# JuliaGaussianProcesses/ApproximateGPs.jl

Hardware: NVIDIA B200
Metric: SVGP ELBO+grad points/sec (FP64) (higher is better)
Workload: dtype f64

## Files before the change

approximategps.jl_b200/csrc/agp.cu:

```cuda
#include <dlfcn.h>
#include <nccl.h>
#include <stdarg.h>
#include <stdio.h>
#include <string.h>

#include <algorithm>
#include <string>
#include <vector>

#include "../../include/agp.h"
#include "dense.cuh"
#include "f32sweep.cuh"
#include "gemm.cuh"
#include "kfun.cuh"
#include "laplace.cuh"
#include "sweep.cuh"

using namespace agp;

static thread_local std::string g_err;
static thread_local int32_t g_err_info = 0;
static int32_t fail(int32_t code, const char* fmt, ...) {
  char buf[1024];
  va_list ap;
// ... 525 lines not shown

template <int MODE>
static int32_t launch_trsm(agp_ctx* c, const TrsmArgs& a, int tiles_n) {
  if ((MODE == TR_KUF_FWD || MODE == TR_KUF_FWD_SCALED) && a.kp.D > 8) return launch_trsm_s<MODE, 3>(c, a, tiles_n);
  return launch_trsm_s<MODE, 4>(c, a, tiles_n);
}

template <int LA, int LB, int S = StageCfg<LA, LB>::stages, class Epi>
static int32_t run_gemm(agp_ctx* c, int tiles_m, int tiles_n, const double* A, int64_t lda, const double* B, int64_t ldb, int K,
                        int kmode, int tmode, const Epi& epi) {
  using Cfg = StageCfg<LA, LB>;
  constexpr int smem_bytes = S * Cfg::bytes;
  GemmArgs g{A, lda, B, ldb, K, kmode, tmode};
  OK((ensure_smem<gemm_kernel<LA, LB, Epi, S>>(c, smem_bytes)));
  dim3 grid(tiles_m, tiles_n);
  if ((kmode == KR_LOWER || kmode == KR_UPPER) && tmode == TS_ALL && tiles_m > 1) {
    static const int env_g = getenv("AGP_SWIZZLE") ? atoi(getenv("AGP_SWIZZLE")) : 0;
    g.swizzle = env_g > 0 ? env_g : std::max(1, c->sms);
    g.tiles_m = tiles_m;
    g.tiles_n = tiles_n;
    grid = dim3(tiles_m * tiles_n, 1);
  }
  gemm_kernel<LA, LB, Epi, S><<<grid, NTHREADS, smem_bytes, c->stream>>>(g, epi);
  LAUNCHED(c);
  KCHECK();
  return AGP_OK;
}

static EpiStore epi_store(double* C, int64_t ldc, bool rowmajor, double alpha = 1.0, double beta = 0.0, int mask = MASK_NONE,
                          double diag_add = 0.0, const double* u = nullptr, const double* v = nullptr, double r1 = 0.0) {
  EpiStore e;
  e.C = C;
  e.ldc = ldc;
  e.rowmajor = rowmajor ? 1 : 0;
  e.alpha = alpha;
  e.beta = beta;
  e.mask = mask;
  e.diag_add = diag_add;
  e.r1u = u;
  e.r1v = v;
  e.r1 = r1;
  return e;
}

static int32_t fill(agp_ctx* c, double* p, int64_t n, double v) {
  if (n <= 0) return AGP_OK;
// ... 976 lines not shown
    } else if (emu_s2 && ncols >= 2048) {
      ProfScope ps(c, PC_GEMM_BTA);
      const int64_t pbytes = (int64_t)Mp * ldc;
      OK(c->q6As.ensure(((int64_t)i8e::S * pbytes + 7) / 8));
      OK(c->sPm.ensure(ldc));
      signed char* qApm = reinterpret_cast<signed char*>(c->q6As.p);
      i8e::transpose_slice_kernel<i8e::S><<<(ncols + 31) / 32, 256, 0, c->stream>>>(c->A.p, ldc, Mp, ncols, qApm, Mp, pbytes, c->sPm.p);
      LAUNCHED(c);
      KCHECK();
      CUtensorMap ma, mb;
      if (!i8e::make_map3(&ma, qApm, Mp, ncols, Mp, pbytes, i8e::EM, i8e::S) ||
          !i8e::make_map3(&mb, reinterpret_cast<signed char*>(c->qBt7.p), Mp, Mp, Mp, MM, i8e::EN, i8e::S))
        return fail(AGP_ERR_CUDA, "cuTensorMapEncodeTiled failed");
      i8e::EpiE2 e2{c->C.p, ldc, c->sPm.p, c->sBt7.p, c->scc_part.p, ldc};
      i8e::Args g8{Mp, i8e::KM_FROM_N, 0, 0};
      OK((ensure_smem<i8e::i8emu_gemm_kernel<i8e::EpiE2>>(c, i8e::SMEM_BYTES)));
      i8e::i8emu_gemm_kernel<i8e::EpiE2><<<dim3(Mp / i8e::EN, ncols / i8e::EM, 1), i8e::E_THREADS, i8e::SMEM_BYTES, c->stream>>>(ma, mb, g8, e2);
      LAUNCHED(c);
      KCHECK();
    } else {
    EpiS2 e2{c->C.p, ldc, c->scc_part.p, ldc};
    {
      ProfScope ps(c, PC_GEMM_BTA);
      OK((run_gemm<A_KM, B_KN>(c, nb, tiles_n, c->Bt_rm.p, Mp, c->A.p, ldc, Mp, KR_UPPER, TS_ALL, e2)));
    }
    }
    PerPointArgs pp{};
    pp.saa = c->saa.p;
    pp.sam = c->sam.p;
    pp.scc_part = c->scc_part.p;
    pp.ldp = ldc;
    pp.nb = st.f32 ? 2 * nb : ((emu_s2 && ncols >= 2048) ? 4 * nb : nb);
    pp.pts = pts;
    pp.y = y ? y + lo : nullptr;
    pp.npts = npts;
    pp.ncols = ncols;
    pp.scale = st.scale;
    pp.mean_const = st.mean_const;
    pp.kp = st.kp;
    pp.lp = st.lp;
    pp.dmu = c->dmu.p;
    pp.dv = c->dv.p;
    pp.mu_out = mu_out ? mu_out + lo : nullptr;
    pp.var_out = var_out ? var_out + lo : nullptr;
    pp.sc_part = c->sc_part.p;
    pp.flag = c->d_flags + 1;
    pp.predict_only = predict ? 1 : 0;
// ... 61 lines not shown
        t5a.kp = st.kp;
        ProfScope ps(c, PC_TRSM_BWD);
        OK(launch_trsm<TR_RHS_BWD>(c, t5a, tiles_n));
      }
      {
        ProfScope ps(c, PC_SYRK);
        const int kchunk = (int)round_up((ncols + c->nsplit - 1) / c->nsplit, t5::TM);
        const int nz = (ncols + kchunk - 1) / kchunk;
        t5::EpiF6 e6{c->Gpart.p, Mp};
        t5::Args g{ncols, t5::KM_SPLIT, kchunk, 1, t5::MnDesc()};
        OK((launch_t5<true, true>(c, dim3(Mp / t5::TM, Mp / t5::TN, nz), fAs, plane, Mp, ncols, fA, plane, Mp, ncols, g, e6)));
      }
      {
        ProfScope ps(c, PC_F32_AUX);
        const int slab = 512, nslab = (ncols + slab - 1) / slab;
        t5::gvec_kernel<<<dim3((Mp / 4 + 255) / 256, nslab), 256, 0, c->stream>>>(fA, fA + plane, Mp, Mp, c->dmu.p, ncols, slab, c->gpart.p, Mp);
        LAUNCHED(c);
        KCHECK();
      }
    } else {
    EpiS4 e4{c->A.p, c->Ab.p, c->As.p, ldc, c->dmu.p, c->dv.p, c->mt.p, c->gpart.p, Mp};
    {
      ProfScope ps(c, PC_GEMM_BC);
      OK((run_gemm<A_KM, B_KN>(c, nb, tiles_n, c->Bt_cm.p, Mp, c->C.p, ldc, Mp, KR_LOWER, TS_ALL, e4)));
    }
    TrsmArgs t5a{};
    t5a.T = c->Ut.p;
    t5a.ldt = Mp;
    t5a.nb = nb;
    t5a.X = c->Ab.p;
    t5a.ldx = ldc;
    t5a.kp = st.kp;
    {
      ProfScope ps(c, PC_TRSM_BWD);
      OK(launch_trsm<TR_RHS_BWD>(c, t5a, tiles_n));
    }
    if (st.f64_emu && Mp >= 768 && ncols >= 2048) {
      ProfScope ps(c, PC_SYRK);
      const int64_t ldk = round_up(ncols, 128), pbytes = (int64_t)Mp * ldk;
      OK(c->q6A.ensure(((int64_t)i8e::S * pbytes + 7) / 8));
      OK(c->q6As.ensure(((int64_t)i8e::S * pbytes + 7) / 8));
      OK(c->s6.ensure(4 * (int64_t)Mp));
      double* sA = c->s6.p;
      double* sAs = c->s6.p + Mp;
      unsigned long long* mx = reinterpret_cast<unsigned long long*>(c->s6.p + 2 * Mp);
      CU(cudaMemsetAsync(mx, 0, sizeof(unsigned long long) * 2 * Mp, c->stream));
      const int seg = 8192;
// ... 8 lines not shown
      c->launches += 4;
      KCHECK();
      CUtensorMap ma, mb;
      if (!i8e::make_map3(&ma, qAs, ldk, Mp, ldk, pbytes, i8e::EM, i8e::S) || !i8e::make_map3(&mb, qA, ldk, Mp, ldk, pbytes, i8e::EN, i8e::S))
        return fail(AGP_ERR_CUDA, "cuTensorMapEncodeTiled failed");
      const int kchunk = 16384, nz = (int)((ldk + kchunk - 1) / kchunk);
      if (nz > c->nsplit) return fail(AGP_ERR_ALLOC, "S6 (INT8): %d slabs of G needed, %d allocated", nz, c->nsplit);
      i8e::EpiE6 e6{c->Gpart.p, Mp, sAs, sA};
      i8e::Args g8{(int)ldk, i8e::KM_SPLIT, kchunk, 1};
      OK((ensure_smem<i8e::i8emu_gemm_kernel<i8e::EpiE6>>(c, i8e::SMEM_BYTES)));
      i8e::i8emu_gemm_kernel<i8e::EpiE6><<<dim3(Mp / i8e::EN, Mp / i8e::EM, nz), i8e::E_THREADS, i8e::SMEM_BYTES, c->stream>>>(ma, mb, g8, e6);
      LAUNCHED(c);
      KCHECK();
    } else {
      ProfScope ps(c, PC_SYRK);
      SyrkArgs s{};
      s.As = c->As.p;
      s.A = c->A.p;
      s.ld = ldc;
      s.ncols = ncols;
      s.kchunk = (int)round_up((ncols + c->nsplit - 1) / c->nsplit, BK);
      s.G = c->Gpart.p;
      s.Mp = Mp;
      using Cfg = StageCfg<A_MK, B_NK>;
      OK((ensure_smem<syrk_kernel>(c, Cfg::smem_bytes)));
      dim3 grid(nb * (nb + 1), c->nsplit);
      syrk_kernel<<<grid, NTHREADS, Cfg::smem_bytes, c->stream>>>(s);
      LAUNCHED(c);
      KCHECK();
    }
    }
    {
      ProfScope ps(c, PC_KGRAD);
      if (kgrad_fast(st)) {
        OK(run_kgrad(c, c->Ab.p, ldc, pts, npts, (npts + 2047) / 2048, c->Kf.p, st.kp.kind != AGP_KERNEL_SE ? c->DKb.p : nullptr));
      } else {
        OK(run_kgrad(c, c->Ab.p, ldc, pts, npts, (npts + 2047) / 2048));
      }
    }
  }
  if (predict || !grad) return AGP_OK;
  sum_slices_kernel<<<(Mp + 255) / 256, 256, 0, c->stream>>>(c->gpart.p, (int)(ldc / BN), Mp, Mp, c->red.p + rl.g);
  LAUNCHED(c);
  KCHECK();
  sum_slices_kernel<<<1024, 256, 0, c->stream>>>(c->Gpart.p, c->nsplit, MM, MM, c->red.p + rl.G);
  LAUNCHED(c);
  KCHECK();
  OK(finish_kgrad(c, c->nslab, 1.0, c->red.p + rl.dZ, c->red.p + rl.theta));
  return AGP_OK;
}
// ... 339 lines not shown
  xbuf.release();
  if (s != AGP_OK) return s;
  if (e != cudaSuccess) return fail(AGP_ERR_CUDA, "mean_and_var: %s", cudaGetErrorString(e));
  return check_step_flags(c, false);
}

static int32_t project_points(agp_ctx* c, const double* X_dev, int n, int ncols, double* Abuf, double* Cbuf, int64_t ldc) {
  SvgpState& st = c->st;
  TrsmArgs t1{};
  t1.T = c->Lt.p;
  t1.ldt = st.Mp;
  t1.nb = st.nb;
  t1.X = Abuf;
  t1.ldx = ldc;
  t1.pts = X_dev;
  t1.npts = n;
  t1.zsp = c->zsp.p;
  t1.mt = c->mt.p;
  t1.saa = c->saa.p;
  t1.sam = c->sam.p;
  t1.kp = st.kp;
  OK(launch_s1(c, t1, ncols / BN));
  EpiS2 e2{Cbuf, ldc, c->scc_part.p, ldc};
  OK((run_gemm<A_KM, B_KN>(c, st.nb, ncols / BN, c->Bt_rm.p, st.Mp, Abuf, ldc, st.Mp, KR_UPPER, TS_ALL, e2)));
  return AGP_OK;
}

constexpr int64_t AGP_MAX_COV_POINTS = 16384;

extern "C" int32_t agp_svgp_mean_and_cov(agp_ctx* c, const agp_svgp_params* p, const double* X1, int64_t n1, const double* X2, int64_t n2,
                                         double* mu1_out, double* cov_out) {
  if (!c || !p || !X1 || n1 < 1 || !cov_out) return fail(AGP_ERR_INVALID, "agp_svgp_mean_and_cov: bad arguments");
  const bool cross = X2 != nullptr;
  if (!cross) n2 = n1;
  if (n2 < 1) return fail(AGP_ERR_INVALID, "agp_svgp_mean_and_cov: bad arguments");
  if (n1 > AGP_MAX_COV_POINTS || n2 > AGP_MAX_COV_POINTS)
    return fail(AGP_ERR_UNSUPPORTED, "full covariances are limited to %lld points per argument (the matrix is dense)", (long long)AGP_MAX_COV_POINTS);
  OK(prepare_step(c, p));
  SvgpState& st = c->st;
  st.scale = 1.0;
  const int D = st.D, Mp = st.Mp;
  const int n1p = (int)round_up(n1, BM), n2p = (int)round_up(n2, BM);
  OK(ensure_sweep_workspace(c, std::max(n1p, n2p), true));
  const int64_t ldc = c->chunk_cols;
  OK(c->px1.ensure((int64_t)n1p * D));
  OK(c->pxs1.ensure((int64_t)n1p * D));
  OK(c->pxn1.ensure(n1p));
// ... 160 lines not shown
```

approximategps.jl_b200/csrc/common.cuh:

```cuda
#pragma once
#include <cuda_runtime.h>
#include <stdint.h>

namespace agp {

constexpr int BM = 128;
constexpr int BN = 64;
constexpr int BK = 16;
constexpr int NTHREADS = 256;
constexpr int PAD = 4;

constexpr int A_KM = 0, A_MK = 1;
constexpr int B_KN = 0, B_NK = 1;

template <int LA>
struct ATile {
  static constexpr int ld = (LA == A_KM) ? (BM + PAD) : (BK + PAD);
  static constexpr int elems = (LA == A_KM) ? BK * (BM + PAD) : BM * (BK + PAD);
};
template <int LB>
struct BTile {
  static constexpr int ld = (LB == B_KN) ? (BN + PAD) : (BK + PAD);
  static constexpr int elems = (LB == B_KN) ? BK * (BN + PAD) : BN * (BK + PAD);
};
// ... 39 lines not shown
      ".reg .pred p;\n"
      "mbarrier.try_wait.parity.shared::cta.b64 p, [%1], %2;\n"
      "selp.u32 %0, 1, 0, p;\n"
      "}\n"
      : "=r"(ok)
      : "r"(s), "r"(parity)
      : "memory");
  return ok != 0;
}
__device__ __forceinline__ void mbar_wait(uint64_t* bar, unsigned parity) {
  while (!mbar_try_wait(bar, parity)) {
  }
}
__device__ __forceinline__ void fence_barrier_init() { asm volatile("fence.mbarrier_init.release.cluster;\n" ::); }
__device__ __forceinline__ void fence_proxy_async() { asm volatile("fence.proxy.async.shared::cta;\n" ::); }
__device__ __forceinline__ void tma_bulk_g2s(void* smem_dst, const void* gmem_src, unsigned bytes, uint64_t* bar) {
  unsigned d = (unsigned)__cvta_generic_to_shared(smem_dst);
  unsigned b = (unsigned)__cvta_generic_to_shared(bar);
  asm volatile("cp.async.bulk.shared::cluster.global.mbarrier::complete_tx::bytes [%0], [%1], %2, [%3];\n" ::"r"(d),
               "l"(gmem_src), "r"(bytes), "r"(b)
               : "memory");
}

template <int LA>
struct ALoad {
  static constexpr int NCH = (BM * BK / 2) / NTHREADS;
  static constexpr int SSTEP = (LA == A_KM) ? (NTHREADS / (BM / 2)) * ATile<LA>::ld : (NTHREADS / (BK / 2)) * ATile<LA>::ld;
  int64_t goff, gstep;
  int soff;
  __device__ __forceinline__ void init(int64_t lda, int tid) {
    if (LA == A_KM) {
      const int k = tid / (BM / 2), mc = tid % (BM / 2);
      goff = (int64_t)k * lda + mc * 2;
      gstep = (int64_t)(NTHREADS / (BM / 2)) * lda;
      soff = k * ATile<LA>::ld + mc * 2;
    } else {
      const int m = tid / (BK / 2), kc = tid % (BK / 2);
      goff = (int64_t)m * lda + kc * 2;
      gstep = (int64_t)(NTHREADS / (BK / 2)) * lda;
      soff = m * ATile<LA>::ld + kc * 2;
    }
  }
  __device__ __forceinline__ void load(double* sA, const double* __restrict__ gtile) const {
    const double* g = gtile + goff;
    double* s = sA + soff;
#pragma unroll
    for (int i = 0; i < NCH; i++) cp_async16(s + i * SSTEP, g + i * gstep);
  }
};
template <int LB>
struct BLoad {
  static constexpr int NCH = (BK * BN / 2) / NTHREADS;
  static constexpr int SSTEP = (LB == B_KN) ? (NTHREADS / (BN / 2)) * BTile<LB>::ld : (NTHREADS / (BK / 2)) * BTile<LB>::ld;
  int64_t goff, gstep;
  int soff;
  __device__ __forceinline__ void init(int64_t ldb, int tid) {
    if (LB == B_KN) {
      const int k = tid / (BN / 2), nc = tid % (BN / 2);
      goff = (int64_t)k * ldb + nc * 2;
      gstep = (int64_t)(NTHREADS / (BN / 2)) * ldb;
      soff = k * BTile<LB>::ld + nc * 2;
    } else {
      const int n = tid / (BK / 2), kc = tid % (BK / 2);
      goff = (int64_t)n * ldb + kc * 2;
      gstep = (int64_t)(NTHREADS / (BK / 2)) * ldb;
      soff = n * BTile<LB>::ld + kc * 2;
    }
  }
  __device__ __forceinline__ void load(double* sB, const double* __restrict__ gtile) const {
    const double* g = gtile + goff;
    double* s = sB + soff;
#pragma unroll
    for (int i = 0; i < NCH; i++) cp_async16(s + i * SSTEP, g + i * gstep);
  }
};

struct ThreadMap {
  int warp, lane, g, t, wm, wn;
  __device__ __forceinline__ ThreadMap() {
    int tid = threadIdx.x;
    warp = tid >> 5;
    lane = tid & 31;
    g = lane >> 2;
    t = lane & 3;
    wm = ((warp < 4) ? warp : 3 - (warp & 3)) * 32;
    wn = (warp >> 2) * 32;
  }
  __device__ __forceinline__ bool tri_active_lower(int krel) const { return krel < wm + 32; }
  __device__ __forceinline__ bool tri_active_upper(int krel) const { return krel + BK > wm; }
  __device__ __forceinline__ int row(int mi) const { return wm + mi * 8 + g; }
  __device__ __forceinline__ int col(int ni, int e) const { return wn + ni * 8 + 2 * t + e; }
};

typedef double Acc[4][4][2];

__device__ __forceinline__ void acc_zero(Acc& acc) {
#pragma unroll
  for (int i = 0; i < 4; i++)
#pragma unroll
    for (int j = 0; j < 4; j++) acc[i][j][0] = acc[i][j][1] = 0.0;
}

template <int LA, int LB>
__device__ __forceinline__ void mma_stage(Acc& acc, const double* __restrict__ sA, const double* __restrict__ sB,
                                          const ThreadMap& tm) {
  constexpr int lda = ATile<LA>::ld, ldb = BTile<LB>::ld;
#pragma unroll
  for (int kk = 0; kk < BK; kk += 4) {
    double a[4], b[4];
#pragma unroll
    for (int mi = 0; mi < 4; mi++)
      a[mi] = (LA == A_KM) ? sA[(kk + tm.t) * lda + tm.wm + mi * 8 + tm.g] : sA[(tm.wm + mi * 8 + tm.g) * lda + kk + tm.t];
#pragma unroll
    for (int ni = 0; ni < 4; ni++)
      b[ni] = (LB == B_KN) ? sB[(kk + tm.t) * ldb + tm.wn + ni * 8 + tm.g] : sB[(tm.wn + ni * 8 + tm.g) * ldb + kk + tm.t];
#pragma unroll
    for (int mi = 0; mi < 4; mi++)
#pragma unroll
      for (int ni = 0; ni < 4; ni++) dmma884(acc[mi][ni], a[mi], b[ni]);
  }
}

__device__ __forceinline__ double block_sum(double v, double* sred ) {
#pragma unroll
  for (int o = 16; o > 0; o >>= 1) v += __shfl_xor_sync(0xffffffffu, v, o);
  int warp = threadIdx.x >> 5, lane = threadIdx.x & 31;
  __syncthreads();
  if (lane == 0) sred[warp] = v;
  __syncthreads();
  double r = 0.0;
  if (threadIdx.x == 0) {
    int nw = (blockDim.x + 31) >> 5;
    for (int w = 0; w < nw; w++) r += sred[w];
  }
  return r;
}

}
```

approximategps.jl_b200/csrc/gemm.cuh:

```cuda
#pragma once
#include "common.cuh"

namespace agp {

constexpr int KR_FULL = 0;
constexpr int KR_LOWER = 1;
constexpr int KR_UPPER = 2;
constexpr int KR_DIAG = 3;
constexpr int TS_ALL = 0;
constexpr int TS_NBLK_LT = 1;
constexpr int TS_NBLK_GT = 2;
constexpr int TS_NBLK_LE = 3;
constexpr int TS_NBLK_LE1 = 4;

struct GemmArgs {
  const double* A;
  int64_t lda;
  const double* B;
  int64_t ldb;
  int K;
  int kmode;
  int tmode;
  int swizzle = 0;
  int tiles_m = 0, tiles_n = 0;
// ... 33 lines not shown
    __syncthreads();
    if (step + S - 1 < nsteps) {
      double* st = smem + slot_issue * Cfg::elems;
      la.load(st, pa);
      lb.load(st + Cfg::a_elems, pb);
      pa += a_step;
      pb += b_step;
    }
    cp_async_commit();
    slot_issue = (slot_issue + 1 == S) ? 0 : slot_issue + 1;
    const double* st = smem + slot_cons * Cfg::elems;
    slot_cons = (slot_cons + 1 == S) ? 0 : slot_cons + 1;
    bool active = whole_active;
    if (tri != TRI_NONE) {
      const int d = step - diag_step;
      if (d >= 0 && d < BM / BK) active = (tri == TRI_LOWER) ? tm.tri_active_lower(d * BK) : tm.tri_active_upper(d * BK);
    }
    if (active) mma_stage<LA, LB>(acc, st, st + Cfg::a_elems, tm);
  }
  cp_async_wait<0>();
  __syncthreads();
}

template <int LA, int LB, class Epi, int S = StageCfg<LA, LB>::stages>
__global__ void __launch_bounds__(NTHREADS, 2) gemm_kernel(GemmArgs g, Epi epi) {
  extern __shared__ __align__(128) double smem[];
  ThreadMap tm;
  int tile_m = blockIdx.x, tile_n = blockIdx.y;
  if (g.swizzle > 0) {
    const int tiles_m = g.tiles_m, tiles_n = g.tiles_n, G = g.swizzle;
    const int id = blockIdx.x;
    const int sg = id / (G * tiles_m);
    const int gw = min(G, tiles_n - sg * G);
    const int r = id - sg * G * tiles_m;
    const int rank = r / gw;
    tile_n = sg * G + r % gw;
    tile_m = (g.kmode == KR_LOWER) ? tiles_m - 1 - rank : rank;
  }
  const int m0 = tile_m * BM, n0 = tile_n * BN;
  const int nblk = n0 / BM;
  if (g.tmode == TS_NBLK_LT && !(nblk < tile_m)) return;
  if (g.tmode == TS_NBLK_GT && !(nblk > tile_m)) return;
  if (g.tmode == TS_NBLK_LE && !(nblk <= tile_m)) return;
  if (g.tmode == TS_NBLK_LE1 && !(nblk <= tile_m + 1)) return;
  int kb = 0, ke = g.K;
  if (g.kmode == KR_LOWER) ke = min(g.K, (tile_m + 1) * BM);
  if (g.kmode == KR_UPPER) kb = tile_m * BM;
  if (g.kmode == KR_DIAG) {
    kb = tile_m * BM;
    ke = kb + BM;
  }
  const double* gA = (LA == A_KM) ? g.A + (int64_t)kb * g.lda + m0 : g.A + (int64_t)m0 * g.lda + kb;
  const double* gB = (LB == B_KN) ? g.B + (int64_t)kb * g.ldb + n0 : g.B + (int64_t)n0 * g.ldb + kb;
  Acc acc;
  acc_zero(acc);
  const int nsteps = (ke - kb) / BK;
  int tri = TRI_NONE, diag_step = 0;
  if (g.kmode == KR_LOWER && ke == (tile_m + 1) * BM) {
    tri = TRI_LOWER;
    diag_step = nsteps - BM / BK;
  } else if (g.kmode == KR_UPPER) {
    tri = TRI_UPPER;
  }
  gemm_mainloop<LA, LB, S>(acc, smem, gA, g.lda, gB, g.ldb, nsteps, tm, tri, diag_step);
  epi(acc, tm, m0, n0, smem);
}

constexpr int MASK_NONE = 0;
constexpr int MASK_LOWER = 1;
constexpr int MASK_PHI = 2;

struct EpiStore {
  double* C;
  int64_t ldc;
  int rowmajor;
  double alpha;
  double beta;
  int mask;
  double diag_add;
  const double* r1u;
  const double* r1v;
  double r1;
  __device__ __forceinline__ void operator()(Acc& acc, const ThreadMap& tm, int m0, int n0, double*) const {
#pragma unroll
    for (int mi = 0; mi < 4; mi++) {
      const int row = m0 + tm.row(mi);
      const double ur = r1u ? r1 * r1u[row] : 0.0;
#pragma unroll
// ... 22 lines not shown
```

approximategps.jl_b200/csrc/sweep.cuh:

```cuda
#pragma once
#include "gemm.cuh"
#include "kfun.cuh"

namespace agp {

constexpr int TR_KUF_FWD = 0, TR_RHS_FWD = 1, TR_RHS_BWD = 2, TR_KUF_FWD_SCALED = 3, TR_RHS_FWD_SUMS = 4;

struct TrsmArgs {
  const double* T;
  int64_t ldt;
  int nb;
  double* X;
  int64_t ldx;
  const double* RHS;
  const double* pts;
  int npts;
  const double* zsp;
  const double* mt;
  double* saa;
  double* sam;
  const double* rowscale;
  const double* dvec;
  double* skd;
  KernelParams kp;
// ... 327 lines not shown
      double k, dk;
      kappa_and_du_gen(kind, u, a.kp.c, k, dk);
      *out = var * k;
      if (outd) {
        *outd = var * dk;
        outd += a.ldx;
      }
    }
  }
  for (int r = rvalid; r < KG_ROWS; r++, out += a.ldx) {
    *out = 0.0;
    if (outd) {
      *outd = 0.0;
      outd += a.ldx;
    }
  }
}

struct EpiS2 {
  double* C;
  int64_t ldc;
  double* scc_part;
  int64_t ldp;
  __device__ __forceinline__ void operator()(Acc& acc, const ThreadMap& tm, int m0, int n0, double* sred) const {
    double pcc[4][2];
#pragma unroll
    for (int ni = 0; ni < 4; ni++) pcc[ni][0] = pcc[ni][1] = 0.0;
#pragma unroll
    for (int mi = 0; mi < 4; mi++) {
      double* cr = C + (int64_t)(m0 + tm.row(mi)) * ldc + n0;
#pragma unroll
      for (int ni = 0; ni < 4; ni++) {
        const double v0 = acc[mi][ni][0], v1 = acc[mi][ni][1];
        *reinterpret_cast<double2*>(cr + tm.col(ni, 0)) = make_double2(v0, v1);
        pcc[ni][0] = fma(v0, v0, pcc[ni][0]);
        pcc[ni][1] = fma(v1, v1, pcc[ni][1]);
      }
    }
#pragma unroll
    for (int ni = 0; ni < 4; ni++)
#pragma unroll
      for (int e = 0; e < 2; e++) {
        double v = pcc[ni][e];
#pragma unroll
        for (int o = 4; o < 32; o <<= 1) v += __shfl_xor_sync(0xffffffffu, v, o);
        if (tm.g == 0) sred[(tm.warp & 3) * 64 + tm.col(ni, e)] = v;
      }
    __syncthreads();
    if (threadIdx.x < BN) {
      const int t = threadIdx.x;
      scc_part[(int64_t)(m0 / BM) * ldp + n0 + t] = ((sred[t] + sred[64 + t]) + sred[128 + t]) + sred[192 + t];
    }
  }
};

struct EpiS4 {
  const double* A;
  double* Ab;
  double* As;
  int64_t ld;
  const double* dmu;
  const double* dv;
  const double* mt;
  double* gpart;
  int64_t ldg;
  __device__ __forceinline__ void operator()(Acc& acc, const ThreadMap& tm, int m0, int n0, double* sred) const {
    double dm[4][2], dvv[4][2];
#pragma unroll
    for (int ni = 0; ni < 4; ni++) {
      const double2 a = *reinterpret_cast<const double2*>(dmu + n0 + tm.col(ni, 0));
      const double2 b = *reinterpret_cast<const double2*>(dv + n0 + tm.col(ni, 0));
      dm[ni][0] = a.x;
      dm[ni][1] = a.y;
      dvv[ni][0] = b.x;
      dvv[ni][1] = b.y;
    }
#pragma unroll
    for (int mi = 0; mi < 4; mi++) {
      const int row = m0 + tm.row(mi);
      const double mtr = mt[row];
      const int64_t off = (int64_t)row * ld + n0;
      double gp = 0.0;
#pragma unroll
      for (int ni = 0; ni < 4; ni++) {
        const int c = tm.col(ni, 0);
        const double2 a = *reinterpret_cast<const double2*>(A + off + c);
        double2 ab, as;
        ab.x = fma(dm[ni][0], mtr, 2.0 * dvv[ni][0] * (acc[mi][ni][0] - a.x));
        ab.y = fma(dm[ni][1], mtr, 2.0 * dvv[ni][1] * (acc[mi][ni][1] - a.y));
        as.x = dvv[ni][0] * a.x;
        as.y = dvv[ni][1] * a.y;
        *reinterpret_cast<double2*>(Ab + off + c) = ab;
        *reinterpret_cast<double2*>(As + off + c) = as;
        gp = fma(dm[ni][0], a.x, gp);
        gp = fma(dm[ni][1], a.y, gp);
      }
      gp += __shfl_xor_sync(0xffffffffu, gp, 1);
      gp += __shfl_xor_sync(0xffffffffu, gp, 2);
      if (tm.t == 0) sred[(tm.warp >> 2) * BM + tm.row(mi)] = gp;
    }
    __syncthreads();
    if (threadIdx.x < BM) gpart[(int64_t)(n0 / BN) * ldg + m0 + threadIdx.x] += sred[threadIdx.x] + sred[BM + threadIdx.x];
  }
};

constexpr int SC_E = 0, SC_DMU = 1, SC_DKXX = 2, SC_DS2 = 3, SC_DC = 4, SC_DS = 5;
constexpr int NSC = SC_DS + MAXD;

struct PerPointArgs {
  const double* saa;
  const double* sam;
  const double* scc_part;
  int64_t ldp;
  int nb;
  const double* pts;
  const double* y;
  int npts;
  int ncols;
  double scale;
  double mean_const;
  KernelParams kp;
  LikParams lp;
  double* dmu;
  double* dv;
// ... 96 lines not shown
  }
}

__global__ void __launch_bounds__(256) scal_reduce_kernel(const double* part, int nblocks, int nsc_used, double* acc) {
  __shared__ double sred[8];
  for (int j = 0; j < nsc_used; j++) {
    double v = 0.0;
    for (int b = threadIdx.x; b < nblocks; b += blockDim.x) v += part[(int64_t)b * NSC + j];
    const double r = block_sum(v, sred);
    if (threadIdx.x == 0) acc[j] += r;
  }
}

struct SyrkArgs {
  const double* As;
  const double* A;
  int64_t ld;
  int ncols;
  int kchunk;
  double* G;
  int Mp;
};

__global__ void __launch_bounds__(NTHREADS, 2) syrk_kernel(SyrkArgs a) {
  extern __shared__ __align__(128) double smem[];
  ThreadMap tm;
  int t = blockIdx.x, ti = 0;
  while (t >= 2 * ti + 2) {
    t -= 2 * ti + 2;
    ti++;
  }
  const int tj = t;
  const int split = blockIdx.y;
  const int kb = split * a.kchunk;
  const int ke = min(a.ncols, kb + a.kchunk);
  if (kb >= ke) return;
  const int m0 = ti * BM, n0 = tj * BN;
  Acc acc;
  acc_zero(acc);
  const bool needed = m0 + tm.wm + 31 >= n0 + tm.wn;
  gemm_mainloop<A_MK, B_NK>(acc, smem, a.As + (int64_t)m0 * a.ld + kb, a.ld, a.A + (int64_t)n0 * a.ld + kb, a.ld,
                            (ke - kb) / BK, tm, TRI_NONE, 0, needed);
  double* G = a.G + (int64_t)split * a.Mp * a.Mp;
#pragma unroll
  for (int mi = 0; mi < 4; mi++)
#pragma unroll
    for (int ni = 0; ni < 4; ni++)
#pragma unroll
      for (int e = 0; e < 2; e++) G[(int64_t)(n0 + tm.col(ni, e)) * a.Mp + m0 + tm.row(mi)] += acc[mi][ni][e];
}

struct KgradArgs {
  const double* Kb;
  const double* Kf;
  const double* DK;
  int64_t ld;
  const double* pts;
  int npts;
  const double* zs;
  const double* zn;
  int slab;
  double* part;
  int stride;
  int Mp;
  KernelParams kp;
};
__host__ __device__ __forceinline__ int kgrad_stride(int D) { return 2 * D + 3 + 2 * MAXC; }
__host__ __device__ __forceinline__ int theta_size(int D) { return 2 + D + 2 * MAXC; }
constexpr int AGP_KERNEL_COMPOSITE = AGP_KERNEL_SUM;

template <int DMAX, int RW, int KIND>
__global__ void __launch_bounds__(256, (DMAX <= 8 && RW == 1) ? 2 : 1) kgrad_kernel(KgradArgs a) {
// ... 312 lines not shown
```

Baseline: 5.483 million.

## Add warp-specialized producer/consumer FP64 GEMM with mbarrier ring for SVGP GEMMs

Introduces a warp-specialized GEMM kernel in which 64 producer threads issue cp.async loads into a multi-stage shared-memory ring guarded by mbarriers, and 128 consumer threads (4 warps, each now owning a 64x32 sub-tile) run the DMMA mainloop. The B^T·A and B·C GEMMs, the projection GEMM and the SYRK kernel all switch to this path, and their epilogues are adapted to the new 8x4 accumulator mapping and a named consumer barrier. The aim is to hide global-load latency by decoupling loads from math. In exchange each consumer thread holds twice as many accumulators, which raises register pressure and may reduce occupancy.

```diff
diff --git a/approximategps.jl_b200/csrc/agp.cu b/approximategps.jl_b200/csrc/agp.cu
--- a/approximategps.jl_b200/csrc/agp.cu
+++ b/approximategps.jl_b200/csrc/agp.cu
@@ -571,6 +571,26 @@
     grid = dim3(tiles_m * tiles_n, 1);
   }
   gemm_kernel<LA, LB, Epi, S><<<grid, NTHREADS, smem_bytes, c->stream>>>(g, epi);
+  LAUNCHED(c);
+  KCHECK();
+  return AGP_OK;
+}
+
+template <class Epi>
+static int32_t run_gemm_ws(agp_ctx* c, int tiles_m, int tiles_n, const double* A, int64_t lda, const double* B, int64_t ldb, int K,
+                           int kmode, const Epi& epi) {
+  constexpr int smem_bytes = ws_smem_bytes<A_KM, B_KN>();
+  GemmArgs g{A, lda, B, ldb, K, kmode, TS_ALL};
+  OK((ensure_smem<gemm_ws_kernel<A_KM, B_KN, Epi>>(c, smem_bytes)));
+  dim3 grid(tiles_m, tiles_n);
+  if ((kmode == KR_LOWER || kmode == KR_UPPER) && tiles_m > 1) {
+    static const int env_g = getenv("AGP_SWIZZLE") ? atoi(getenv("AGP_SWIZZLE")) : 0;
+    g.swizzle = env_g > 0 ? env_g : std::max(1, c->sms);
+    g.tiles_m = tiles_m;
+    g.tiles_n = tiles_n;
+    grid = dim3(tiles_m * tiles_n, 1);
+  }
+  gemm_ws_kernel<A_KM, B_KN, Epi><<<grid, WS_THREADS, smem_bytes, c->stream>>>(g, epi);
   LAUNCHED(c);
   KCHECK();
   return AGP_OK;
@@ -1593,7 +1613,7 @@
     EpiS2 e2{c->C.p, ldc, c->scc_part.p, ldc};
     {
       ProfScope ps(c, PC_GEMM_BTA);
-      OK((run_gemm<A_KM, B_KN>(c, nb, tiles_n, c->Bt_rm.p, Mp, c->A.p, ldc, Mp, KR_UPPER, TS_ALL, e2)));
+      OK((run_gemm_ws(c, nb, tiles_n, c->Bt_rm.p, Mp, c->A.p, ldc, Mp, KR_UPPER, e2)));
     }
     }
     PerPointArgs pp{};
@@ -1701,7 +1721,7 @@
     EpiS4 e4{c->A.p, c->Ab.p, c->As.p, ldc, c->dmu.p, c->dv.p, c->mt.p, c->gpart.p, Mp};
     {
       ProfScope ps(c, PC_GEMM_BC);
-      OK((run_gemm<A_KM, B_KN>(c, nb, tiles_n, c->Bt_cm.p, Mp, c->C.p, ldc, Mp, KR_LOWER, TS_ALL, e4)));
+      OK((run_gemm_ws(c, nb, tiles_n, c->Bt_cm.p, Mp, c->C.p, ldc, Mp, KR_LOWER, e4)));
     }
     TrsmArgs t5a{};
     t5a.T = c->Ut.p;
@@ -1756,10 +1776,10 @@
       s.kchunk = (int)round_up((ncols + c->nsplit - 1) / c->nsplit, BK);
       s.G = c->Gpart.p;
       s.Mp = Mp;
-      using Cfg = StageCfg<A_MK, B_NK>;
-      OK((ensure_smem<syrk_kernel>(c, Cfg::smem_bytes)));
+      constexpr int smem_bytes = ws_smem_bytes<A_MK, B_NK>();
+      OK((ensure_smem<syrk_kernel>(c, smem_bytes)));
       dim3 grid(nb * (nb + 1), c->nsplit);
-      syrk_kernel<<<grid, NTHREADS, Cfg::smem_bytes, c->stream>>>(s);
+      syrk_kernel<<<grid, WS_THREADS, smem_bytes, c->stream>>>(s);
       LAUNCHED(c);
       KCHECK();
     }
@@ -2145,7 +2165,7 @@
   t1.kp = st.kp;
   OK(launch_s1(c, t1, ncols / BN));
   EpiS2 e2{Cbuf, ldc, c->scc_part.p, ldc};
-  OK((run_gemm<A_KM, B_KN>(c, st.nb, ncols / BN, c->Bt_rm.p, st.Mp, Abuf, ldc, st.Mp, KR_UPPER, TS_ALL, e2)));
+  OK((run_gemm_ws(c, st.nb, ncols / BN, c->Bt_rm.p, st.Mp, Abuf, ldc, st.Mp, KR_UPPER, e2)));
   return AGP_OK;
 }
 
diff --git a/approximategps.jl_b200/csrc/common.cuh b/approximategps.jl_b200/csrc/common.cuh
--- a/approximategps.jl_b200/csrc/common.cuh
+++ b/approximategps.jl_b200/csrc/common.cuh
@@ -85,22 +85,23 @@
                : "memory");
 }
 
-template <int LA>
+template <int LA, int NT = NTHREADS>
 struct ALoad {
-  static constexpr int NCH = (BM * BK / 2) / NTHREADS;
-  static constexpr int SSTEP = (LA == A_KM) ? (NTHREADS / (BM / 2)) * ATile<LA>::ld : (NTHREADS / (BK / 2)) * ATile<LA>::ld;
+  static constexpr int NCH = (BM * BK / 2) / NT;
+  static constexpr int SSTEP = (LA == A_KM) ? (NT / (BM / 2)) * ATile<LA>::ld : (NT / (BK / 2)) * ATile<LA>::ld;
+  static_assert(NT >= BM / 2, "one pass of the threads covers whole tile rows");
   int64_t goff, gstep;
   int soff;
   __device__ __forceinline__ void init(int64_t lda, int tid) {
     if (LA == A_KM) {
       const int k = tid / (BM / 2), mc = tid % (BM / 2);
       goff = (int64_t)k * lda + mc * 2;
-      gstep = (int64_t)(NTHREADS / (BM / 2)) * lda;
+      gstep = (int64_t)(NT / (BM / 2)) * lda;
       soff = k * ATile<LA>::ld + mc * 2;
     } else {
       const int m = tid / (BK / 2), kc = tid % (BK / 2);
       goff = (int64_t)m * lda + kc * 2;
-      gstep = (int64_t)(NTHREADS / (BK / 2)) * lda;
+      gstep = (int64_t)(NT / (BK / 2)) * lda;
       soff = m * ATile<LA>::ld + kc * 2;
     }
   }
@@ -111,22 +112,22 @@
     for (int i = 0; i < NCH; i++) cp_async16(s + i * SSTEP, g + i * gstep);
   }
 };
-template <int LB>
+template <int LB, int NT = NTHREADS>
 struct BLoad {
-  static constexpr int NCH = (BK * BN / 2) / NTHREADS;
-  static constexpr int SSTEP = (LB == B_KN) ? (NTHREADS / (BN / 2)) * BTile<LB>::ld : (NTHREADS / (BK / 2)) * BTile<LB>::ld;
+  static constexpr int NCH = (BK * BN / 2) / NT;
+  static constexpr int SSTEP = (LB == B_KN) ? (NT / (BN / 2)) * BTile<LB>::ld : (NT / (BK / 2)) * BTile<LB>::ld;
   int64_t goff, gstep;
   int soff;
   __device__ __forceinline__ void init(int64_t ldb, int tid) {
     if (LB == B_KN) {
       const int k = tid / (BN / 2), nc = tid % (BN / 2);
       goff = (int64_t)k * ldb + nc * 2;
-      gstep = (int64_t)(NTHREADS / (BN / 2)) * ldb;
+      gstep = (int64_t)(NT / (BN / 2)) * ldb;
       soff = k * BTile<LB>::ld + nc * 2;
     } else {
       const int n = tid / (BK / 2), kc = tid % (BK / 2);
       goff = (int64_t)n * ldb + kc * 2;
-      gstep = (int64_t)(NTHREADS / (BK / 2)) * ldb;
+      gstep = (int64_t)(NT / (BK / 2)) * ldb;
       soff = n * BTile<LB>::ld + kc * 2;
     }
   }
@@ -164,21 +165,89 @@
     for (int j = 0; j < 4; j++) acc[i][j][0] = acc[i][j][1] = 0.0;
 }
 
-template <int LA, int LB>
-__device__ __forceinline__ void mma_stage(Acc& acc, const double* __restrict__ sA, const double* __restrict__ sB,
-                                          const ThreadMap& tm) {
+constexpr int WS_CONSUMERS = 128;
+constexpr int WS_PRODUCERS = 64;
+constexpr int WS_THREADS = WS_CONSUMERS + WS_PRODUCERS;
+
+__device__ __forceinline__ void mbar_arrive(uint64_t* bar) {
+  asm volatile("mbarrier.arrive.shared::cta.b64 _, [%0];\n" ::"r"((unsigned)__cvta_generic_to_shared(bar)) : "memory");
+}
+__device__ __forceinline__ void cp_async_mbar_arrive_noinc(uint64_t* bar) {
+  asm volatile("cp.async.mbarrier.arrive.noinc.shared::cta.b64 [%0];\n" ::"r"((unsigned)__cvta_generic_to_shared(bar)) : "memory");
+}
+__device__ __forceinline__ void consumer_sync() { asm volatile("bar.sync 1, %0;\n" ::"n"(WS_CONSUMERS) : "memory"); }
+
+template <int S>
+struct Ring {
+  static constexpr int bar_bytes = 2 * S * 8;
+  uint64_t* full;
+  uint64_t* empty;
+  int slot;
+  unsigned phase;
+  __device__ __forceinline__ void init(uint64_t* bars) {
+    full = bars;
+    empty = bars + S;
+    slot = 0;
+    phase = 0;
+    if (threadIdx.x == 0) {
+      for (int s = 0; s < S; s++) {
+        mbar_init(&full[s], WS_PRODUCERS);
+        mbar_init(&empty[s], WS_CONSUMERS / 32);
+      }
+    }
+  }
+  __device__ __forceinline__ void advance() {
+    if (++slot == S) {
+      slot = 0;
+      phase ^= 1;
+    }
+  }
+  __device__ __forceinline__ void acquire() { mbar_wait(&empty[slot], phase ^ 1); }
+  __device__ __forceinline__ void commit() {
+    cp_async_mbar_arrive_noinc(&full[slot]);
+    advance();
+  }
+  __device__ __forceinline__ void wait() { mbar_wait(&full[slot], phase); }
+  __device__ __forceinline__ void release() {
+    __syncwarp();
+    if ((threadIdx.x & 31) == 0) mbar_arrive(&empty[slot]);
+    advance();
+  }
+};
+
+struct WsMap {
+  int warp, lane, g, t, wm, wn;
+  __device__ __forceinline__ WsMap() {
+    int tid = threadIdx.x;
+    warp = tid >> 5;
+    lane = tid & 31;
+    g = lane >> 2;
+    t = lane & 3;
+    wm = (warp & 1) * 64;
+    wn = (warp >> 1) * 32;
+  }
+  __device__ __forceinline__ bool tri_active_lower(int krel) const { return krel < wm + 64; }
+  __device__ __forceinline__ bool tri_active_upper(int krel) const { return krel + BK > wm; }
+  __device__ __forceinline__ int row(int mi) const { return wm + mi * 8 + g; }
+  __device__ __forceinline__ int col(int ni, int e) const { return wn + ni * 8 + 2 * t + e; }
+};
+typedef double AccW[8][4][2];
+
+template <int LA, int LB, int MI, class Map>
+__device__ __forceinline__ void mma_stage(double (&acc)[MI][4][2], const double* __restrict__ sA, const double* __restrict__ sB,
+                                          const Map& tm) {
   constexpr int lda = ATile<LA>::ld, ldb = BTile<LB>::ld;
 #pragma unroll
   for (int kk = 0; kk < BK; kk += 4) {
-    double a[4], b[4];
-#pragma unroll
-    for (int mi = 0; mi < 4; mi++)
+    double a[MI], b[4];
+#pragma unroll
+    for (int mi = 0; mi < MI; mi++)
       a[mi] = (LA == A_KM) ? sA[(kk + tm.t) * lda + tm.wm + mi * 8 + tm.g] : sA[(tm.wm + mi * 8 + tm.g) * lda + kk + tm.t];
 #pragma unroll
     for (int ni = 0; ni < 4; ni++)
       b[ni] = (LB == B_KN) ? sB[(kk + tm.t) * ldb + tm.wn + ni * 8 + tm.g] : sB[(tm.wn + ni * 8 + tm.g) * ldb + kk + tm.t];
 #pragma unroll
-    for (int mi = 0; mi < 4; mi++)
+    for (int mi = 0; mi < MI; mi++)
 #pragma unroll
       for (int ni = 0; ni < 4; ni++) dmma884(acc[mi][ni], a[mi], b[ni]);
   }
diff --git a/approximategps.jl_b200/csrc/gemm.cuh b/approximategps.jl_b200/csrc/gemm.cuh
--- a/approximategps.jl_b200/csrc/gemm.cuh
+++ b/approximategps.jl_b200/csrc/gemm.cuh
@@ -79,48 +79,127 @@
   __syncthreads();
 }
 
+struct GemmTile {
+  int m0, n0, nsteps, tri, diag_step;
+  int64_t a_off, b_off;
+  template <int LA, int LB>
+  __device__ __forceinline__ bool decode(const GemmArgs& g) {
+    int tile_m = blockIdx.x, tile_n = blockIdx.y;
+    if (g.swizzle > 0) {
+      const int tiles_m = g.tiles_m, tiles_n = g.tiles_n, G = g.swizzle;
+      const int id = blockIdx.x;
+      const int sg = id / (G * tiles_m);
+      const int gw = min(G, tiles_n - sg * G);
+      const int r = id - sg * G * tiles_m;
+      const int rank = r / gw;
+      tile_n = sg * G + r % gw;
+      tile_m = (g.kmode == KR_LOWER) ? tiles_m - 1 - rank : rank;
+    }
+    m0 = tile_m * BM;
+    n0 = tile_n * BN;
+    const int nblk = n0 / BM;
+    if (g.tmode == TS_NBLK_LT && !(nblk < tile_m)) return false;
+    if (g.tmode == TS_NBLK_GT && !(nblk > tile_m)) return false;
+    if (g.tmode == TS_NBLK_LE && !(nblk <= tile_m)) return false;
+    if (g.tmode == TS_NBLK_LE1 && !(nblk <= tile_m + 1)) return false;
+    int kb = 0, ke = g.K;
+    if (g.kmode == KR_LOWER) ke = min(g.K, (tile_m + 1) * BM);
+    if (g.kmode == KR_UPPER) kb = tile_m * BM;
+    if (g.kmode == KR_DIAG) {
+      kb = tile_m * BM;
+      ke = kb + BM;
+    }
+    a_off = (LA == A_KM) ? (int64_t)kb * g.lda + m0 : (int64_t)m0 * g.lda + kb;
+    b_off = (LB == B_KN) ? (int64_t)kb * g.ldb + n0 : (int64_t)n0 * g.ldb + kb;
+    nsteps = (ke - kb) / BK;
+    tri = TRI_NONE;
+    diag_step = 0;
+    if (g.kmode == KR_LOWER && ke == (tile_m + 1) * BM) {
+      tri = TRI_LOWER;
+      diag_step = nsteps - BM / BK;
+    } else if (g.kmode == KR_UPPER) {
+      tri = TRI_UPPER;
+    }
+    return true;
+  }
+};
+
 template <int LA, int LB, class Epi, int S = StageCfg<LA, LB>::stages>
 __global__ void __launch_bounds__(NTHREADS, 2) gemm_kernel(GemmArgs g, Epi epi) {
   extern __shared__ __align__(128) double smem[];
   ThreadMap tm;
-  int tile_m = blockIdx.x, tile_n = blockIdx.y;
-  if (g.swizzle > 0) {
-    const int tiles_m = g.tiles_m, tiles_n = g.tiles_n, G = g.swizzle;
-    const int id = blockIdx.x;
-    const int sg = id / (G * tiles_m);
-    const int gw = min(G, tiles_n - sg * G);
-    const int r = id - sg * G * tiles_m;
-    const int rank = r / gw;
-    tile_n = sg * G + r % gw;
-    tile_m = (g.kmode == KR_LOWER) ? tiles_m - 1 - rank : rank;
-  }
-  const int m0 = tile_m * BM, n0 = tile_n * BN;
-  const int nblk = n0 / BM;
-  if (g.tmode == TS_NBLK_LT && !(nblk < tile_m)) return;
-  if (g.tmode == TS_NBLK_GT && !(nblk > tile_m)) return;
-  if (g.tmode == TS_NBLK_LE && !(nblk <= tile_m)) return;
-  if (g.tmode == TS_NBLK_LE1 && !(nblk <= tile_m + 1)) return;
-  int kb = 0, ke = g.K;
-  if (g.kmode == KR_LOWER) ke = min(g.K, (tile_m + 1) * BM);
-  if (g.kmode == KR_UPPER) kb = tile_m * BM;
-  if (g.kmode == KR_DIAG) {
-    kb = tile_m * BM;
-    ke = kb + BM;
-  }
-  const double* gA = (LA == A_KM) ? g.A + (int64_t)kb * g.lda + m0 : g.A + (int64_t)m0 * g.lda + kb;
-  const double* gB = (LB == B_KN) ? g.B + (int64_t)kb * g.ldb + n0 : g.B + (int64_t)n0 * g.ldb + kb;
+  GemmTile t;
+  if (!t.decode<LA, LB>(g)) return;
   Acc acc;
   acc_zero(acc);
-  const int nsteps = (ke - kb) / BK;
-  int tri = TRI_NONE, diag_step = 0;
-  if (g.kmode == KR_LOWER && ke == (tile_m + 1) * BM) {
-    tri = TRI_LOWER;
-    diag_step = nsteps - BM / BK;
-  } else if (g.kmode == KR_UPPER) {
-    tri = TRI_UPPER;
-  }
-  gemm_mainloop<LA, LB, S>(acc, smem, gA, g.lda, gB, g.ldb, nsteps, tm, tri, diag_step);
-  epi(acc, tm, m0, n0, smem);
+  gemm_mainloop<LA, LB, S>(acc, smem, g.A + t.a_off, g.lda, g.B + t.b_off, g.ldb, t.nsteps, tm, t.tri, t.diag_step);
+  epi(acc, tm, t.m0, t.n0, smem);
+}
+
+template <int LA, int LB, int S = StageCfg<LA, LB>::stages>
+constexpr int ws_smem_bytes() {
+  return S * StageCfg<LA, LB>::bytes + Ring<S>::bar_bytes;
+}
+template <int LA, int LB, int S>
+__device__ __forceinline__ void ws_produce(Ring<S>& ring, double* smem, const double* __restrict__ gA, int64_t lda,
+                                           const double* __restrict__ gB, int64_t ldb, int nsteps) {
+  using Cfg = StageCfg<LA, LB>;
+  const int p = threadIdx.x - WS_CONSUMERS;
+  ALoad<LA, WS_PRODUCERS> la;
+  BLoad<LB, WS_PRODUCERS> lb;
+  la.init(lda, p);
+  lb.init(ldb, p);
+  const int64_t a_step = (LA == A_KM) ? (int64_t)BK * lda : (int64_t)BK;
+  const int64_t b_step = (LB == B_KN) ? (int64_t)BK * ldb : (int64_t)BK;
+  for (int step = 0; step < nsteps; step++) {
+    ring.acquire();
+    double* st = smem + ring.slot * Cfg::elems;
+    la.load(st, gA);
+    lb.load(st + Cfg::a_elems, gB);
+    ring.commit();
+    gA += a_step;
+    gB += b_step;
+  }
+  asm volatile("cp.async.wait_all;\n" ::: "memory");
+}
+template <int LA, int LB, int S>
+__device__ __forceinline__ void ws_consume(AccW& acc, Ring<S>& ring, const double* smem, int nsteps, const WsMap& tm,
+                                           int tri = TRI_NONE, int diag_step = 0, bool whole_active = true) {
+  using Cfg = StageCfg<LA, LB>;
+  for (int step = 0; step < nsteps; step++) {
+    ring.wait();
+    const double* st = smem + ring.slot * Cfg::elems;
+    bool active = whole_active;
+    if (tri != TRI_NONE) {
+      const int d = step - diag_step;
+      if (d >= 0 && d < BM / BK) active = (tri == TRI_LOWER) ? tm.tri_active_lower(d * BK) : tm.tri_active_upper(d * BK);
+    }
+    if (active) mma_stage<LA, LB>(acc, st, st + Cfg::a_elems, tm);
+    ring.release();
+  }
+  consumer_sync();
+}
+
+template <int LA, int LB, class Epi, int S = StageCfg<LA, LB>::stages>
+__global__ void __launch_bounds__(WS_THREADS, 2) gemm_ws_kernel(GemmArgs g, Epi epi) {
+  extern __shared__ __align__(128) double smem[];
+  GemmTile t;
+  if (!t.decode<LA, LB>(g)) return;
+  Ring<S> ring;
+  ring.init(reinterpret_cast<uint64_t*>(smem + S * StageCfg<LA, LB>::elems));
+  __syncthreads();
+  if (threadIdx.x >= WS_CONSUMERS) {
+    ws_produce<LA, LB, S>(ring, smem, g.A + t.a_off, g.lda, g.B + t.b_off, g.ldb, t.nsteps);
+    return;
+  }
+  WsMap tm;
+  AccW acc;
+#pragma unroll
+  for (int i = 0; i < 8; i++)
+#pragma unroll
+    for (int j = 0; j < 4; j++) acc[i][j][0] = acc[i][j][1] = 0.0;
+  ws_consume<LA, LB, S>(acc, ring, smem, t.nsteps, tm, t.tri, t.diag_step);
+  epi(acc, tm, t.m0, t.n0, smem);
 }
 
 constexpr int MASK_NONE = 0;
diff --git a/approximategps.jl_b200/csrc/sweep.cuh b/approximategps.jl_b200/csrc/sweep.cuh
--- a/approximategps.jl_b200/csrc/sweep.cuh
+++ b/approximategps.jl_b200/csrc/sweep.cuh
@@ -373,31 +373,36 @@
   int64_t ldc;
   double* scc_part;
   int64_t ldp;
-  __device__ __forceinline__ void operator()(Acc& acc, const ThreadMap& tm, int m0, int n0, double* sred) const {
-    double pcc[4][2];
-#pragma unroll
-    for (int ni = 0; ni < 4; ni++) pcc[ni][0] = pcc[ni][1] = 0.0;
-#pragma unroll
-    for (int mi = 0; mi < 4; mi++) {
-      double* cr = C + (int64_t)(m0 + tm.row(mi)) * ldc + n0;
-#pragma unroll
-      for (int ni = 0; ni < 4; ni++) {
-        const double v0 = acc[mi][ni][0], v1 = acc[mi][ni][1];
-        *reinterpret_cast<double2*>(cr + tm.col(ni, 0)) = make_double2(v0, v1);
-        pcc[ni][0] = fma(v0, v0, pcc[ni][0]);
-        pcc[ni][1] = fma(v1, v1, pcc[ni][1]);
-      }
-    }
-#pragma unroll
-    for (int ni = 0; ni < 4; ni++)
-#pragma unroll
-      for (int e = 0; e < 2; e++) {
-        double v = pcc[ni][e];
-#pragma unroll
-        for (int o = 4; o < 32; o <<= 1) v += __shfl_xor_sync(0xffffffffu, v, o);
-        if (tm.g == 0) sred[(tm.warp & 3) * 64 + tm.col(ni, e)] = v;
-      }
-    __syncthreads();
+  __device__ __forceinline__ void operator()(AccW& acc, const WsMap& tm, int m0, int n0, double* sred) const {
+#pragma unroll
+    for (int h = 0; h < 2; h++) {
+      double pcc[4][2];
+#pragma unroll
+      for (int ni = 0; ni < 4; ni++) pcc[ni][0] = pcc[ni][1] = 0.0;
+#pragma unroll
+      for (int mi = 4 * h; mi < 4 * h + 4; mi++) {
+        double* cr = C + (int64_t)(m0 + tm.row(mi)) * ldc + n0;
+#pragma unroll
+        for (int ni = 0; ni < 4; ni++) {
+          const double v0 = acc[mi][ni][0], v1 = acc[mi][ni][1];
+          *reinterpret_cast<double2*>(cr + tm.col(ni, 0)) = make_double2(v0, v1);
+          pcc[ni][0] = fma(v0, v0, pcc[ni][0]);
+          pcc[ni][1] = fma(v1, v1, pcc[ni][1]);
+        }
+      }
+      const int q = (tm.wm >> 5) + h;
+      const int slot = tm.wn == 0 ? q : 3 - q;
+#pragma unroll
+      for (int ni = 0; ni < 4; ni++)
+#pragma unroll
+        for (int e = 0; e < 2; e++) {
+          double v = pcc[ni][e];
+#pragma unroll
+          for (int o = 4; o < 32; o <<= 1) v += __shfl_xor_sync(0xffffffffu, v, o);
+          if (tm.g == 0) sred[slot * 64 + tm.col(ni, e)] = v;
+        }
+    }
+    consumer_sync();
     if (threadIdx.x < BN) {
       const int t = threadIdx.x;
       scc_part[(int64_t)(m0 / BM) * ldp + n0 + t] = ((sred[t] + sred[64 + t]) + sred[128 + t]) + sred[192 + t];
@@ -415,42 +420,36 @@
   const double* mt;
   double* gpart;
   int64_t ldg;
-  __device__ __forceinline__ void operator()(Acc& acc, const ThreadMap& tm, int m0, int n0, double* sred) const {
-    double dm[4][2], dvv[4][2];
-#pragma unroll
-    for (int ni = 0; ni < 4; ni++) {
-      const double2 a = *reinterpret_cast<const double2*>(dmu + n0 + tm.col(ni, 0));
-      const double2 b = *reinterpret_cast<const double2*>(dv + n0 + tm.col(ni, 0));
-      dm[ni][0] = a.x;
-      dm[ni][1] = a.y;
-      dvv[ni][0] = b.x;
-      dvv[ni][1] = b.y;
-    }
-#pragma unroll
-    for (int mi = 0; mi < 4; mi++) {
+  __device__ __forceinline__ void operator()(AccW& acc, const WsMap& tm, int m0, int n0, double* sred) const {
+    const int c0 = n0 + tm.col(0, 0);
+    const int64_t off0 = (int64_t)(m0 + tm.row(0)) * ld + c0;
+#pragma unroll
+    for (int mi = 0; mi < 8; mi++) {
       const int row = m0 + tm.row(mi);
       const double mtr = mt[row];
-      const int64_t off = (int64_t)row * ld + n0;
+      const int64_t off = off0 + (int64_t)(mi * 8) * ld;
       double gp = 0.0;
 #pragma unroll
       for (int ni = 0; ni < 4; ni++) {
-        const int c = tm.col(ni, 0);
+        const int c = ni * 8;
+        const double2 dm = *reinterpret_cast<const double2*>(dmu + c0 + c);
+        const double2 dvv = *reinterpret_cast<const double2*>(dv + c0 + c);
         const double2 a = *reinterpret_cast<const double2*>(A + off + c);
         double2 ab, as;
-        ab.x = fma(dm[ni][0], mtr, 2.0 * dvv[ni][0] * (acc[mi][ni][0] - a.x));
-        ab.y = fma(dm[ni][1], mtr, 2.0 * dvv[ni][1] * (acc[mi][ni][1] - a.y));
-        as.x = dvv[ni][0] * a.x;
-        as.y = dvv[ni][1] * a.y;
+        ab.x = fma(dm.x, mtr, 2.0 * dvv.x * (acc[mi][ni][0] - a.x));
+        ab.y = fma(dm.y, mtr, 2.0 * dvv.y * (acc[mi][ni][1] - a.y));
+        as.x = dvv.x * a.x;
+        as.y = dvv.y * a.y;
         *reinterpret_cast<double2*>(Ab + off + c) = ab;
         *reinterpret_cast<double2*>(As + off + c) = as;
-        gp = fma(dm[ni][0], a.x, gp);
-        gp = fma(dm[ni][1], a.y, gp);
+        gp = fma(dm.x, a.x, gp);
+        gp = fma(dm.y, a.y, gp);
       }
       gp += __shfl_xor_sync(0xffffffffu, gp, 1);
       gp += __shfl_xor_sync(0xffffffffu, gp, 2);
-      if (tm.t == 0) sred[(tm.warp >> 2) * BM + tm.row(mi)] = gp;
-    }
-    __syncthreads();
+      if (tm.t == 0) sred[(tm.wn >> 5) * BM + tm.row(mi)] = gp;
+    }
+    consumer_sync();
     if (threadIdx.x < BM) gpart[(int64_t)(n0 / BN) * ldg + m0 + threadIdx.x] += sred[threadIdx.x] + sred[BM + threadIdx.x];
   }
 };
@@ -593,9 +592,9 @@
   int Mp;
 };
 
-__global__ void __launch_bounds__(NTHREADS, 2) syrk_kernel(SyrkArgs a) {
+__global__ void __launch_bounds__(WS_THREADS, 2) syrk_kernel(SyrkArgs a) {
   extern __shared__ __align__(128) double smem[];
-  ThreadMap tm;
+  constexpr int S = StageCfg<A_MK, B_NK>::stages;
   int t = blockIdx.x, ti = 0;
   while (t >= 2 * ti + 2) {
     t -= 2 * ti + 2;
@@ -607,18 +606,30 @@
   const int ke = min(a.ncols, kb + a.kchunk);
   if (kb >= ke) return;
   const int m0 = ti * BM, n0 = tj * BN;
-  Acc acc;
-  acc_zero(acc);
-  const bool needed = m0 + tm.wm + 31 >= n0 + tm.wn;
-  gemm_mainloop<A_MK, B_NK>(acc, smem, a.As + (int64_t)m0 * a.ld + kb, a.ld, a.A + (int64_t)n0 * a.ld + kb, a.ld,
-                            (ke - kb) / BK, tm, TRI_NONE, 0, needed);
+  Ring<S> ring;
+  ring.init(reinterpret_cast<uint64_t*>(smem + S * StageCfg<A_MK, B_NK>::elems));
+  __syncthreads();
+  if (threadIdx.x >= WS_CONSUMERS) {
+    ws_produce<A_MK, B_NK, S>(ring, smem, a.As + (int64_t)m0 * a.ld + kb, a.ld, a.A + (int64_t)n0 * a.ld + kb, a.ld, (ke - kb) / BK);
+    return;
+  }
+  WsMap tm;
+  AccW acc;
+#pragma unroll
+  for (int i = 0; i < 8; i++)
+#pragma unroll
+    for (int j = 0; j < 4; j++) acc[i][j][0] = acc[i][j][1] = 0.0;
+  const bool needed = m0 + tm.wm + 63 >= n0 + tm.wn;
+  ws_consume<A_MK, B_NK, S>(acc, ring, smem, (ke - kb) / BK, tm, TRI_NONE, 0, needed);
   double* G = a.G + (int64_t)split * a.Mp * a.Mp;
 #pragma unroll
-  for (int mi = 0; mi < 4; mi++)
+  for (int mi = 0; mi < 8; mi++) {
+    const bool blk = m0 + tm.wm + (mi >> 2) * 32 + 31 >= n0 + tm.wn;
 #pragma unroll
     for (int ni = 0; ni < 4; ni++)
 #pragma unroll
-      for (int e = 0; e < 2; e++) G[(int64_t)(n0 + tm.col(ni, e)) * a.Mp + m0 + tm.row(mi)] += acc[mi][ni][e];
+      for (int e = 0; e < 2; e++) G[(int64_t)(n0 + tm.col(ni, e)) * a.Mp + m0 + tm.row(mi)] += blk ? acc[mi][ni][e] : 0.0;
+  }
 }
 
 struct KgradArgs {
```

Result: slower. 5.344 million (median of 6 runs) (-2.5%).
